# socom20/speech-cloner

Measured on AMD Instinct MI355X. Metric: mel frames/sec, higher is better.
Workload: dtype bf16; 1 GPU; full: STFT+mel front-end on batch 32 x 4 s @ 16 kHz (configs[1] input) -> 64 windows of 400 frames -> encoder (enc_14 weights) + decoder (hp/decoder_cfg_d.json sizes, random init), 64 windows per launch, independent steps pipelined over 10 HIP streams; batch=32, samples=64000, windows=64, model_dtype=bfloat16, streams=10, parallelism=utterance-sharded x1, no collective

## Files before the change

### speech-cloner_amd/csrc/vc_highway.hip

```cpp
#include "vc_device.h"

using vc::f32x16, vc::f32x4, vc::bf16x8, vc::bf16x4;

namespace {

constexpr int HW_BM = 128;
constexpr int HW_MAX_LAYERS = 8;
constexpr int HW_RING = 4;

struct HwChainArgs {
    const __bf16* X;
    __bf16* Y;
    int32_t M, ldx, ldy, n_layers;
    const __bf16* W[HW_MAX_LAYERS];
    const float* bias[HW_MAX_LAYERS];
    const __bf16* PW;
    const float* Pbias;
    float* P;
    int32_t NP, ldp;
};

template <int H>
__device__ __forceinline__ void hw_tile(const bf16x8* pw, const bf16x8* next, const char* xrow, int lh, int x15,
                                        bf16x8 (&ring)[HW_RING][2], f32x16 (&acc)[4][2]) {
    constexpr int KS = H / 16, RB = 2 * H;
#pragma unroll
    for (int i = 0; i < 4; ++i)
#pragma unroll
        for (int c = 0; c < 2; ++c)
#pragma unroll
            for (int r = 0; r < 16; ++r) acc[i][c][r] = 0.0f;
    bf16x8 xf[2][4];
#pragma unroll
    for (int i = 0; i < 4; ++i) xf[0][i] = *reinterpret_cast<const bf16x8*>(xrow + i * 32 * RB + ((lh ^ x15) << 4));
#pragma unroll 1
    for (int s0 = 0; s0 < KS; s0 += HW_RING) {
        const bf16x8* src = (s0 + HW_RING < KS) ? pw + (size_t)(s0 + HW_RING) * 128 : next;
#pragma unroll
        for (int u = 0; u < HW_RING; ++u) {
            const int s = s0 + u, cb = u & 1;
            if (s + 1 < KS) {
#pragma unroll
                for (int i = 0; i < 4; ++i)
                    xf[cb ^ 1][i] = *reinterpret_cast<const bf16x8*>(xrow + i * 32 * RB + (((2 * (s + 1) + lh) ^ x15) << 4));
            }
            const bf16x8 w0 = ring[u][0], w1 = ring[u][1];
            if (src) {
                ring[u][0] = src[u * 128];
                ring[u][1] = src[u * 128 + 64];
            }
#pragma unroll
            for (int i = 0; i < 4; ++i) {
                acc[i][0] = __builtin_amdgcn_mfma_f32_32x32x16_bf16(w0, xf[cb][i], acc[i][0], 0, 0, 0);
                acc[i][1] = __builtin_amdgcn_mfma_f32_32x32x16_bf16(w1, xf[cb][i], acc[i][1], 0, 0, 0);
            }
        }
    }
}

template <int H>
__global__ void __launch_bounds__(2 * H, H == 256 ? 1 : 2)
highway_chain_kernel(HwChainArgs a) {
    constexpr int NT = 2 * H, KS = H / 16, RB = 2 * H, NS = H / 8;
    extern __shared__ __attribute__((aligned(16))) char smem[];
    const int tid = threadIdx.x, lane = tid & 63;
    const int w = __builtin_amdgcn_readfirstlane(tid >> 6);
    const int li = lane & 31, lh = lane >> 5, x15 = li & 15;
    const int m0 = blockIdx.x * HW_BM;

    for (int idx = tid; idx < HW_BM * NS; idx += NT) {
        const int row = idx / NS, slot = idx - row * NS;
        const int gm = min(m0 + row, a.M - 1);
        const bf16x8 v = *reinterpret_cast<const bf16x8*>(a.X + (size_t)gm * a.ldx + slot * 8);
        *reinterpret_cast<bf16x8*>(smem + row * RB + ((slot ^ (row & 15)) << 4)) = v;
    }

    float* bias_s = reinterpret_cast<float*>(smem + 2 * HW_BM * RB);
    for (int idx = tid; idx < a.n_layers * 2 * H; idx += NT) {
        const int l = idx / (2 * H);
        bias_s[idx] = a.bias[l][idx - l * 2 * H];
    }

    bf16x8 wr[HW_RING][2];
    auto wptr = [&](int layer, int s) {
        return reinterpret_cast<const bf16x8*>(a.W[layer]) + ((size_t)(w * KS + s) * 2) * 64 + lane;
    };
    if (a.n_layers > 0) {
#pragma unroll
        for (int s = 0; s < HW_RING; ++s) {
            const bf16x8* p = wptr(0, s);
            wr[s][0] = p[0];
            wr[s][1] = p[64];
        }
    }
    __syncthreads();

    for (int layer = 0; layer < a.n_layers; ++layer) {
        const char* cur = smem + (layer & 1) * (HW_BM * RB);
        char* nxt = smem + ((layer & 1) ^ 1) * (HW_BM * RB);
        const bool more = layer + 1 < a.n_layers;
        f32x16 acc[4][2];
        const bf16x8* nextw = more ? wptr(layer + 1, 0) : (a.PW && w < a.NP / 64 ? reinterpret_cast<const bf16x8*>(a.PW) + ((size_t)w * KS * 2) * 64 + lane : nullptr);
        hw_tile<H>(wptr(layer, 0), nextw, cur + li * RB, lh, x15, wr, acc);
        f32x4 bH[4], bT[4];
#pragma unroll
        for (int q = 0; q < 4; ++q) {
            bH[q] = *reinterpret_cast<const f32x4*>(bias_s + layer * 2 * H + w * 64 + 8 * q + 4 * lh);
            bT[q] = *reinterpret_cast<const f32x4*>(bias_s + layer * 2 * H + w * 64 + 32 + 8 * q + 4 * lh);
        }
#pragma unroll
        for (int i = 0; i < 4; ++i) {
#pragma unroll
            for (int q = 0; q < 4; ++q) {
                const int off = (i * 32 + li) * RB + (((4 * w + q) ^ x15) << 4) + lh * 8;
                const bf16x4 xin = *reinterpret_cast<const bf16x4*>(cur + off);
                bf16x4 o;
#pragma unroll
                for (int e = 0; e < 4; ++e) {
                    o[e] = (__bf16)vc::highway_gate(acc[i][0][4 * q + e] + bH[q][e], acc[i][1][4 * q + e] + bT[q][e], (float)xin[e]);
                }
                *reinterpret_cast<bf16x4*>(nxt + off) = o;
            }
        }
        __syncthreads();
    }

    const char* fin = smem + (a.n_layers & 1) * (HW_BM * RB);
    if (a.PW) {
        constexpr int NW = 2 * H / 64;
        const int ngroups = a.NP / 64;
        const char* xrow = fin + li * RB;
        char* const stg = smem + ((a.n_layers & 1) ^ 1) * (HW_BM * RB) + w * 8192;
        static_assert((2 * H / 64) * 8192 <= HW_BM * 2 * H, "a 32 x 64 float32 sub-tile per wave fits the idle buffer");
        if (a.n_layers == 0 && w < ngroups) {
            const bf16x8* p0 = reinterpret_cast<const bf16x8*>(a.PW) + ((size_t)w * KS * 2) * 64 + lane;
#pragma unroll
            for (int s = 0; s < HW_RING; ++s) { wr[s][0] = p0[s * 128]; wr[s][1] = p0[s * 128 + 64]; }
        }
        for (int grp = w; grp < ngroups; grp += NW) {
            const bf16x8* pw = reinterpret_cast<const bf16x8*>(a.PW) + ((size_t)grp * KS * 2) * 64 + lane;
            const bf16x8* nextw = (grp + NW < ngroups) ? pw + (size_t)NW * KS * 128 : nullptr;
            f32x16 acc[4][2];
            hw_tile<H>(pw, nextw, xrow, lh, x15, wr, acc);
#pragma unroll
            for (int c = 0; c < 2; ++c)
#pragma unroll
                for (int q = 0; q < 4; ++q) {
                    const f32x4 bb = *reinterpret_cast<const f32x4*>(a.Pbias + grp * 64 + c * 32 + 8 * q + 4 * lh);
#pragma unroll
                    for (int i = 0; i < 4; ++i)
#pragma unroll
                        for (int e = 0; e < 4; ++e) acc[i][c][4 * q + e] += bb[e];
                }
#pragma unroll
            for (int i = 0; i < 4; ++i) {
#pragma unroll
                for (int c = 0; c < 2; ++c)
#pragma unroll
                    for (int q = 0; q < 4; ++q) {
                        f32x4 o;
#pragma unroll
                        for (int e = 0; e < 4; ++e) o[e] = acc[i][c][4 * q + e];
                        *reinterpret_cast<f32x4*>(stg + li * 256 + (((c * 8 + 2 * q + lh) ^ x15) << 4)) = o;
                    }
#pragma unroll 2
                for (int j = 0; j < 8; ++j) {
                    const int row = j * 4 + (lane >> 4), ch = lane & 15;
                    const f32x4 v = *reinterpret_cast<const f32x4*>(stg + row * 256 + ((ch ^ (row & 15)) << 4));
                    const int gm = m0 + i * 32 + row;
                    if (gm < a.M) *reinterpret_cast<f32x4*>(a.P + (size_t)gm * a.ldp + grp * 64 + ch * 4) = v;
                }
            }
        }
    }
    if (a.Y == nullptr) return;
    for (int idx = tid; idx < HW_BM * NS; idx += NT) {
        const int row = idx / NS, slot = idx - row * NS;
        const int gm = m0 + row;
        if (gm < a.M)
            *reinterpret_cast<bf16x8*>(a.Y + (size_t)gm * a.ldy + slot * 8) =
                *reinterpret_cast<const bf16x8*>(fin + row * RB + ((slot ^ (row & 15)) << 4));
    }
}

template <int H> int launch_chain(const HwChainArgs& a, hipStream_t st) {
    constexpr int LDS = 2 * HW_BM * 2 * H + HW_MAX_LAYERS * 2 * H * 4;
    if (int rc = vc::allow_dynamic_lds<highway_chain_kernel<H>>(LDS)) return rc;
    hipLaunchKernelGGL(highway_chain_kernel<H>, dim3((a.M + HW_BM - 1) / HW_BM), dim3(2 * H), LDS, st, a);
    VC_HIP_CHECK(hipGetLastError());
    return VC_OK;
}

__global__ void __launch_bounds__(256)
highway_pack_kernel(const __bf16* Bt, int ncols, int H, __bf16* packed) {
    const int KS = H / 16, total = (ncols / 64) * KS * 2 * 64 * 8;
    for (int idx = blockIdx.x * 256 + threadIdx.x; idx < total; idx += gridDim.x * 256) {
        int r = idx;
        const int j = r & 7; r >>= 3;
        const int lane = r & 63; r >>= 6;
        const int c = r & 1; r >>= 1;
        const int s = r % KS;
        const int w = r / KS;
        packed[idx] = Bt[(size_t)(w * 64 + c * 32 + (lane & 31)) * H + s * 16 + (lane >> 5) * 8 + j];
    }
}

}

extern "C" {

int vc_highway_pack(const void* d_Bt, int32_t n_cols, int32_t H, void* d_packed, void* stream) {
    VC_REQUIRE(d_Bt && d_packed && (H == 128 || H == 256) && n_cols > 0 && n_cols % 64 == 0,
               "vc_highway_pack: H must be 128 or 256 and n_cols a multiple of 64");
    hipLaunchKernelGGL(highway_pack_kernel, dim3(128), dim3(256), 0, static_cast<hipStream_t>(stream),
                       static_cast<const __bf16*>(d_Bt), n_cols, H, static_cast<__bf16*>(d_packed));
    VC_HIP_CHECK(hipGetLastError());
    return VC_OK;
}

int vc_highway_chain(const void* d_X, int32_t M, int32_t H, int32_t ldx, int32_t n_layers, const void* const* d_packed,
                     const float* const* d_bias, void* d_Y, int32_t ldy, const void* d_proj_packed,
                     const float* d_proj_bias, int32_t n_proj, float* d_P, int32_t ldp, void* stream) {
    VC_REQUIRE(d_X && d_packed && d_bias && (d_Y || d_proj_packed), "vc_highway_chain: NULL argument");
    if (d_proj_packed)
        VC_REQUIRE(d_proj_bias && d_P && n_proj > 0 && n_proj % 64 == 0 && ldp >= n_proj && ldp % 4 == 0 &&
                       ((reinterpret_cast<uintptr_t>(d_proj_packed) | reinterpret_cast<uintptr_t>(d_proj_bias) |
                         reinterpret_cast<uintptr_t>(d_P)) & 15) == 0,
                   "vc_highway_chain: projection tail needs bias, output, n_proj %% 64 == 0, 16-byte aligned operands");
    VC_REQUIRE(H == 128 || H == 256, "vc_highway_chain: H must be 128 or 256 (got %d)", H);
    VC_REQUIRE(M > 0 && n_layers >= 0 && n_layers <= HW_MAX_LAYERS, "vc_highway_chain: bad M / n_layers");
    VC_REQUIRE(ldx >= H && ldx % 8 == 0 && (!d_Y || (ldy >= H && ldy % 8 == 0)), "vc_highway_chain: ldx / ldy must be multiples of 8 and >= H");
    VC_REQUIRE(((reinterpret_cast<uintptr_t>(d_X) | reinterpret_cast<uintptr_t>(d_Y)) & 15) == 0, "vc_highway_chain: X / Y must be 16-byte aligned");
    HwChainArgs a;
    a.X = static_cast<const __bf16*>(d_X); a.Y = static_cast<__bf16*>(d_Y);
    a.M = M; a.ldx = ldx; a.ldy = ldy; a.n_layers = n_layers;
    a.PW = static_cast<const __bf16*>(d_proj_packed); a.Pbias = d_proj_bias; a.P = d_P; a.NP = n_proj; a.ldp = ldp;
    for (int l = 0; l < n_layers; ++l) {
        VC_REQUIRE(d_packed[l] && d_bias[l] && (reinterpret_cast<uintptr_t>(d_packed[l]) & 15) == 0 &&
                       (reinterpret_cast<uintptr_t>(d_bias[l]) & 15) == 0, "vc_highway_chain: layer %d operands NULL or misaligned", l);
        a.W[l] = static_cast<const __bf16*>(d_packed[l]);
        a.bias[l] = d_bias[l];
    }
    hipStream_t st = static_cast<hipStream_t>(stream);
    return H == 256 ? launch_chain<256>(a, st) : launch_chain<128>(a, st);
}

}
```

Baseline: 14.30 million frames/s.

## Deepen weight prefetch ring for H=256 and hoist global loads in highway chain

Makes the weight register ring depth depend on H (8 for H=256, else 4) and switches to byte-offset addressing with unconditional prefetch, so there is no per-step branch. Activation and bias loads are issued into registers before the LDS stores, so they overlap with the first weight fill. The projection bias is now fetched once per lane before the tile and broadcast through LDS, and the Y write-back is moved ahead of the projection loop. The deeper ring raises register pressure, the unconditional prefetch re-reads the current weights when nothing comes next, and the bias staging reads LDS without an explicit wave-level barrier.

```diff
diff --git a/speech-cloner_amd/csrc/vc_highway.hip b/speech-cloner_amd/csrc/vc_highway.hip
--- a/speech-cloner_amd/csrc/vc_highway.hip
+++ b/speech-cloner_amd/csrc/vc_highway.hip
@@ -1,12 +1,13 @@
 #include "vc_device.h"
 
 using vc::f32x16, vc::f32x4, vc::bf16x8, vc::bf16x4;
+typedef float __attribute__((may_alias)) f32_alias;
 
 namespace {
 
 constexpr int HW_BM = 128;
 constexpr int HW_MAX_LAYERS = 8;
-constexpr int HW_RING = 4;
+constexpr int hw_ring_depth(int H) { return H == 256 ? 8 : 4; }
 
 struct HwChainArgs {
     const __bf16* X;
@@ -20,10 +21,11 @@
     int32_t NP, ldp;
 };
 
-template <int H>
-__device__ __forceinline__ void hw_tile(const bf16x8* pw, const bf16x8* next, const char* xrow, int lh, int x15,
-                                        bf16x8 (&ring)[HW_RING][2], f32x16 (&acc)[4][2]) {
+template <int H, int D>
+__device__ __forceinline__ void hw_tile(const char* pw, const char* next, unsigned lane16, const char* xrow, int lh, int x15,
+                                        bf16x8 (&ring)[D][2], f32x16 (&acc)[4][2]) {
     constexpr int KS = H / 16, RB = 2 * H;
+    static_assert(D >= 2 && D % 2 == 0 && KS % D == 0, "a tile is a whole number of ring fills; the activation double buffer alternates per step");
 #pragma unroll
     for (int i = 0; i < 4; ++i)
 #pragma unroll
@@ -34,10 +36,10 @@
 #pragma unroll
     for (int i = 0; i < 4; ++i) xf[0][i] = *reinterpret_cast<const bf16x8*>(xrow + i * 32 * RB + ((lh ^ x15) << 4));
 #pragma unroll 1
-    for (int s0 = 0; s0 < KS; s0 += HW_RING) {
-        const bf16x8* src = (s0 + HW_RING < KS) ? pw + (size_t)(s0 + HW_RING) * 128 : next;
-#pragma unroll
-        for (int u = 0; u < HW_RING; ++u) {
+    for (int s0 = 0; s0 < KS; s0 += D) {
+        const char* src = (s0 + D < KS) ? pw + (size_t)(s0 + D) * 2048 : (next ? next : pw);
+#pragma unroll
+        for (int u = 0; u < D; ++u) {
             const int s = s0 + u, cb = u & 1;
             if (s + 1 < KS) {
 #pragma unroll
@@ -45,10 +47,8 @@
                     xf[cb ^ 1][i] = *reinterpret_cast<const bf16x8*>(xrow + i * 32 * RB + (((2 * (s + 1) + lh) ^ x15) << 4));
             }
             const bf16x8 w0 = ring[u][0], w1 = ring[u][1];
-            if (src) {
-                ring[u][0] = src[u * 128];
-                ring[u][1] = src[u * 128 + 64];
-            }
+            ring[u][0] = *reinterpret_cast<const bf16x8*>(src + lane16 + u * 2048);
+            ring[u][1] = *reinterpret_cast<const bf16x8*>(src + lane16 + u * 2048 + 1024);
 #pragma unroll
             for (int i = 0; i < 4; ++i) {
                 acc[i][0] = __builtin_amdgcn_mfma_f32_32x32x16_bf16(w0, xf[cb][i], acc[i][0], 0, 0, 0);
@@ -61,38 +61,46 @@
 template <int H>
 __global__ void __launch_bounds__(2 * H, H == 256 ? 1 : 2)
 highway_chain_kernel(HwChainArgs a) {
-    constexpr int NT = 2 * H, KS = H / 16, RB = 2 * H, NS = H / 8;
+    constexpr int NT = 2 * H, KS = H / 16, RB = 2 * H, NS = H / 8, D = hw_ring_depth(H);
     extern __shared__ __attribute__((aligned(16))) char smem[];
     const int tid = threadIdx.x, lane = tid & 63;
     const int w = __builtin_amdgcn_readfirstlane(tid >> 6);
     const int li = lane & 31, lh = lane >> 5, x15 = li & 15;
     const int m0 = blockIdx.x * HW_BM;
 
-    for (int idx = tid; idx < HW_BM * NS; idx += NT) {
-        const int row = idx / NS, slot = idx - row * NS;
+    constexpr int NX = HW_BM * NS / NT;
+    static_assert(NX * NT == HW_BM * NS, "every thread carries the same number of 16-byte slots");
+    bf16x8 xv[NX];
+#pragma unroll
+    for (int k = 0; k < NX; ++k) {
+        const int idx = tid + k * NT, row = idx / NS, slot = idx - row * NS;
         const int gm = min(m0 + row, a.M - 1);
-        const bf16x8 v = *reinterpret_cast<const bf16x8*>(a.X + (size_t)gm * a.ldx + slot * 8);
-        *reinterpret_cast<bf16x8*>(smem + row * RB + ((slot ^ (row & 15)) << 4)) = v;
-    }
-
+        xv[k] = *reinterpret_cast<const bf16x8*>(a.X + (size_t)gm * a.ldx + slot * 8);
+    }
     float* bias_s = reinterpret_cast<float*>(smem + 2 * HW_BM * RB);
-    for (int idx = tid; idx < a.n_layers * 2 * H; idx += NT) {
-        const int l = idx / (2 * H);
-        bias_s[idx] = a.bias[l][idx - l * 2 * H];
-    }
-
-    bf16x8 wr[HW_RING][2];
-    auto wptr = [&](int layer, int s) {
-        return reinterpret_cast<const bf16x8*>(a.W[layer]) + ((size_t)(w * KS + s) * 2) * 64 + lane;
+    float bv[HW_MAX_LAYERS];
+#pragma unroll
+    for (int l = 0; l < HW_MAX_LAYERS; ++l) bv[l] = l < a.n_layers ? a.bias[l][tid] : 0.0f;
+    bf16x8 wr[D][2];
+    const unsigned lane16 = lane * 16;
+    auto wptr = [&](int layer) { return reinterpret_cast<const char*>(a.W[layer]) + (size_t)w * KS * 2048; };
+    auto tptr = [&](int grp) { return reinterpret_cast<const char*>(a.PW) + (size_t)grp * KS * 2048; };
+    auto fill = [&](const char* p) {
+#pragma unroll
+        for (int s = 0; s < D; ++s) {
+            wr[s][0] = *reinterpret_cast<const bf16x8*>(p + lane16 + s * 2048);
+            wr[s][1] = *reinterpret_cast<const bf16x8*>(p + lane16 + s * 2048 + 1024);
+        }
     };
-    if (a.n_layers > 0) {
-#pragma unroll
-        for (int s = 0; s < HW_RING; ++s) {
-            const bf16x8* p = wptr(0, s);
-            wr[s][0] = p[0];
-            wr[s][1] = p[64];
-        }
-    }
+    if (a.n_layers > 0) fill(wptr(0));
+#pragma unroll
+    for (int k = 0; k < NX; ++k) {
+        const int idx = tid + k * NT, row = idx / NS, slot = idx - row * NS;
+        *reinterpret_cast<bf16x8*>(smem + row * RB + ((slot ^ (row & 15)) << 4)) = xv[k];
+    }
+#pragma unroll
+    for (int l = 0; l < HW_MAX_LAYERS; ++l)
+        if (l < a.n_layers) bias_s[l * 2 * H + tid] = bv[l];
     __syncthreads();
 
     for (int layer = 0; layer < a.n_layers; ++layer) {
@@ -100,8 +108,8 @@
         char* nxt = smem + ((layer & 1) ^ 1) * (HW_BM * RB);
         const bool more = layer + 1 < a.n_layers;
         f32x16 acc[4][2];
-        const bf16x8* nextw = more ? wptr(layer + 1, 0) : (a.PW && w < a.NP / 64 ? reinterpret_cast<const bf16x8*>(a.PW) + ((size_t)w * KS * 2) * 64 + lane : nullptr);
-        hw_tile<H>(wptr(layer, 0), nextw, cur + li * RB, lh, x15, wr, acc);
+        const char* nextw = more ? wptr(layer + 1) : (a.PW && w < a.NP / 64 ? tptr(w) : nullptr);
+        hw_tile<H, D>(wptr(layer), nextw, lane16, cur + li * RB, lh, x15, wr, acc);
         f32x4 bH[4], bT[4];
 #pragma unroll
         for (int q = 0; q < 4; ++q) {
@@ -126,27 +134,33 @@
     }
 
     const char* fin = smem + (a.n_layers & 1) * (HW_BM * RB);
+    if (a.Y) {
+        for (int idx = tid; idx < HW_BM * NS; idx += NT) {
+            const int row = idx / NS, slot = idx - row * NS;
+            const int gm = m0 + row;
+            if (gm < a.M)
+                *reinterpret_cast<bf16x8*>(a.Y + (size_t)gm * a.ldy + slot * 8) =
+                    *reinterpret_cast<const bf16x8*>(fin + row * RB + ((slot ^ (row & 15)) << 4));
+        }
+    }
     if (a.PW) {
         constexpr int NW = 2 * H / 64;
         const int ngroups = a.NP / 64;
         const char* xrow = fin + li * RB;
         char* const stg = smem + ((a.n_layers & 1) ^ 1) * (HW_BM * RB) + w * 8192;
         static_assert((2 * H / 64) * 8192 <= HW_BM * 2 * H, "a 32 x 64 float32 sub-tile per wave fits the idle buffer");
-        if (a.n_layers == 0 && w < ngroups) {
-            const bf16x8* p0 = reinterpret_cast<const bf16x8*>(a.PW) + ((size_t)w * KS * 2) * 64 + lane;
-#pragma unroll
-            for (int s = 0; s < HW_RING; ++s) { wr[s][0] = p0[s * 128]; wr[s][1] = p0[s * 128 + 64]; }
-        }
+        if (a.n_layers == 0 && w < ngroups) fill(tptr(w));
         for (int grp = w; grp < ngroups; grp += NW) {
-            const bf16x8* pw = reinterpret_cast<const bf16x8*>(a.PW) + ((size_t)grp * KS * 2) * 64 + lane;
-            const bf16x8* nextw = (grp + NW < ngroups) ? pw + (size_t)NW * KS * 128 : nullptr;
+            const char* nextw = (grp + NW < ngroups) ? tptr(grp + NW) : nullptr;
             f32x16 acc[4][2];
-            hw_tile<H>(pw, nextw, xrow, lh, x15, wr, acc);
+            const float pb = a.Pbias[grp * 64 + lane];
+            hw_tile<H, D>(tptr(grp), nextw, lane16, xrow, lh, x15, wr, acc);
+            reinterpret_cast<f32_alias*>(stg)[lane] = pb;
 #pragma unroll
             for (int c = 0; c < 2; ++c)
 #pragma unroll
                 for (int q = 0; q < 4; ++q) {
-                    const f32x4 bb = *reinterpret_cast<const f32x4*>(a.Pbias + grp * 64 + c * 32 + 8 * q + 4 * lh);
+                    const f32x4 bb = *reinterpret_cast<const f32x4*>(stg + (c * 32 + 8 * q + 4 * lh) * 4);
 #pragma unroll
                     for (int i = 0; i < 4; ++i)
 #pragma unroll
@@ -172,14 +186,6 @@
                 }
             }
         }
-    }
-    if (a.Y == nullptr) return;
-    for (int idx = tid; idx < HW_BM * NS; idx += NT) {
-        const int row = idx / NS, slot = idx - row * NS;
-        const int gm = m0 + row;
-        if (gm < a.M)
-            *reinterpret_cast<bf16x8*>(a.Y + (size_t)gm * a.ldy + slot * 8) =
-                *reinterpret_cast<const bf16x8*>(fin + row * RB + ((slot ^ (row & 15)) << 4));
     }
 }
 
```

Result: no change. 14.21 million frames/s (-0.6%).
